# jseppanen/azalea

Hardware: AMD Instinct MI355X
Metric: mcts_sims_per_sec (higher is better)
Workload: dtype f16x3 (fp32 operands split hi+lo f16, fp32 accumulate)

## Files before the change

### azalea_amd/csrc/net_kernels.hip

```cpp
#include "net_priv.h"
#include "tower_tiles.h"

#ifndef AZX_NET_ABLATE
#define AZX_NET_ABLATE 0
#endif
#ifndef AZX_SAT_TRACK
#define AZX_SAT_TRACK 1
#endif

#include <cmath>
#include <cstdio>
#include <cstdlib>
#include <cstring>
#include <map>
#include <string>
#include <type_traits>
#include <utility>
#include <vector>

typedef float f32x16 __attribute__((ext_vector_type(16)));

static thread_local std::string g_net_err;
const char *azx_net_error() { return g_net_err.c_str(); }

// ... 47 lines not shown
            Xb[(size_t)rows * LDW + ncells * LDW + c] = 0.0f;
        }
    }
    __syncthreads();

    const int li = lane & 31, lh = lane >> 5;
    int ry[MTW], rx[MTW];
    bool rvalid[MTW];
#pragma unroll
    for (int m = 0; m < MTW; ++m) {
        const int r = (ms * MTW + m) * 32 + li;
        rvalid[m] = r < ncells;
        ry[m] = r / N;
        rx[m] = r - ry[m] * N;
    }

    for (int layer = 0; layer < P.layers; ++layer) {
        const float *src = (layer & 1) ? Y : X;
        float *dst = (layer & 1) ? X : Y;
        f32x16 acc[MTW][NTW];
#pragma unroll
        for (int m = 0; m < MTW; ++m)
#pragma unroll
            for (int n = 0; n < NTW; ++n)
#pragma unroll
                for (int r = 0; r < 16; ++r) acc[m][n][r] = 0.0f;

        const float4 *wl = reinterpret_cast<const float4 *>(P.Wp) +
                           (size_t)layer * 9 * (C / 8) * NT * 64;
        for (int tap = 0; tap < 9; ++tap) {
            const int dy = tap / 3 - 1, dx = tap % 3 - 1;
            int aoff[MTW];
#pragma unroll
            for (int m = 0; m < MTW; ++m) {
                const int yy = ry[m] + dy, xx = rx[m] + dx;
                const bool ok = rvalid[m] && yy >= 0 && yy < N && xx >= 0 && xx < N;
                aoff[m] = (ok ? (yy * N + xx) : ncells) * LDW + 4 * lh;
            }
            const float4 *wt = wl + (size_t)tap * (C / 8) * NT * 64;
#pragma unroll 2
            for (int q = 0; q < C / 8; ++q) {
                float4 bfrag[NTW];
#pragma unroll
                for (int n = 0; n < NTW; ++n)
                    bfrag[n] = wt[((size_t)q * NT + (ns * NTW + n)) * 64 + lane];
                float4 afrag[MTW];
#pragma unroll
                for (int m = 0; m < MTW; ++m)
                    afrag[m] = *reinterpret_cast<const float4 *>(src + aoff[m] + 8 * q);
#pragma unroll
                for (int m = 0; m < MTW; ++m)
#pragma unroll
                    for (int n = 0; n < NTW; ++n) {
                        acc[m][n] = __builtin_amdgcn_mfma_f32_32x32x2f32(afrag[m].x, bfrag[n].x, acc[m][n], 0, 0, 0);
                        acc[m][n] = __builtin_amdgcn_mfma_f32_32x32x2f32(afrag[m].y, bfrag[n].y, acc[m][n], 0, 0, 0);
                        acc[m][n] = __builtin_amdgcn_mfma_f32_32x32x2f32(afrag[m].z, bfrag[n].z, acc[m][n], 0, 0, 0);
                        acc[m][n] = __builtin_amdgcn_mfma_f32_32x32x2f32(afrag[m].w, bfrag[n].w, acc[m][n], 0, 0, 0);
                    }
            }
        }
        const bool residual = (layer & 1) != 0;
#pragma unroll
        for (int n = 0; n < NTW; ++n) {
            const int co = (ns * NTW + n) * 32 + li;
            const float bb = P.bias[layer * C + co];
#pragma unroll
            for (int m = 0; m < MTW; ++m) {
#pragma unroll
                for (int r = 0; r < 16; ++r) {
                    const int row = (ms * MTW + m) * 32 + (r & 3) + 8 * (r >> 2) + 4 * lh;
                    if (row < ncells) {
                        float v = acc[m][n][r] + bb;
                        if (residual) v += dst[row * LDW + co];
                        dst[row * LDW + co] = fmaxf(v, 0.0f);
                    }
                }
            }
        }
        __syncthreads();
    }

    for (int b = 0; b < BPB; ++b) {
        const int e = e0 + b;
        if (e >= n_eval) break;
        const float *Xb = lds + (size_t)b * 2 * rows * LDW;
        float4 *out = reinterpret_cast<float4 *>(act_out + (size_t)e * ncells * C);
        for (int idx = tid; idx < ncells * (C / 4); idx += 256) {
            const int pos = idx / (C / 4), c4 = idx - pos * (C / 4);
            out[idx] = *reinterpret_cast<const float4 *>(Xb + pos * LDW + 4 * c4);
        }
    }
}


typedef _Float16 f16x8 __attribute__((ext_vector_type(8)));

__device__ __forceinline__ void split_f16(float v, _Float16 &hi, _Float16 &lo) {
    hi = (_Float16)v;
    lo = (_Float16)(v - (float)hi);
}
__device__ __forceinline__ void split2_f16(float a, float b, uint32_t &hpk, uint32_t &lpk) {
    float la, lb;
    asm("v_cvt_pk_f16_f32 %0, %1, %2" : "=v"(hpk) : "v"(a), "v"(b));
    asm("v_fma_mix_f32 %0, %1, -1.0, %2 op_sel_hi:[1,0,0]" : "=v"(la) : "v"(hpk), "v"(a));
    asm("v_fma_mix_f32 %0, %1, -1.0, %2 op_sel:[1,0,0] op_sel_hi:[1,0,0]" : "=v"(lb) : "v"(hpk), "v"(b));
    asm("v_cvt_pk_f16_f32 %0, %1, %2" : "=v"(lpk) : "v"(la), "v"(lb));
#if AZX_LO_BITS < 10
    lpk = (lpk + LO_RND * 0x10001u) & (LO_MASK * 0x10001u);
#endif
}

#ifdef AZX_NET_STAMP
__device__ unsigned long long g_tower_stamp[10];
#define NT_DECL unsigned long long nt_last = __builtin_amdgcn_s_memtime(), nt_acc[8] = {0, 0, 0, 0, 0, 0, 0, 0}; const unsigned long long nt_rt0 = __builtin_amdgcn_s_memrealtime();
__device__ unsigned long long g_tower_trace[3 * 32768];
#define NT_MARK(r) { const unsigned long long nt_now = __builtin_amdgcn_s_memtime(); nt_acc[r] += nt_now - nt_last; nt_last = nt_now; }
#define NT_FLUSH if (tid == 0) { for (int r_ = 0; r_ < 7; ++r_) atomicAdd(&g_tower_stamp[r_], nt_acc[r_]); atomicAdd(&g_tower_stamp[7], 1ull); atomicAdd(&g_tower_stamp[8], __builtin_amdgcn_s_memrealtime() - nt_rt0); \
    if (blockIdx.x < 32768) { const unsigned hw = __builtin_amdgcn_s_getreg((31 << 11) | 4), xc = __builtin_amdgcn_s_getreg((31 << 11) | 20); \
        g_tower_trace[3 * blockIdx.x] = ((unsigned long long)(xc & 0xf) << 8) | (((hw >> 13) & 7) << 5) | (((hw >> 12) & 1) << 4) | ((hw >> 8) & 0xf); \
        g_tower_trace[3 * blockIdx.x + 1] = nt_rt0; g_tower_trace[3 * blockIdx.x + 2] = __builtin_amdgcn_s_memrealtime(); } }
__device__ unsigned long long g_wide_stamp[10];
#define WT_FLUSH if (lane == 0) { for (int r_ = 0; r_ < 7; ++r_) atomicAdd(&g_wide_stamp[r_], nt_acc[r_]); atomicAdd(&g_wide_stamp[7], 1ull); \
    atomicAdd(&g_wide_stamp[8], __builtin_amdgcn_s_memrealtime() - nt_rt0); }
#else
#define NT_DECL
#define NT_MARK(r)
#define NT_FLUSH
#define WT_FLUSH
#endif

#ifndef F16X3_BPB
#define F16X3_BPB 2
#endif
#ifndef AZX_S16_FENCE
#define AZX_S16_FENCE 1
#endif
typedef float f32x4 __attribute__((ext_vector_type(4)));

__global__ __launch_bounds__(F16X3_BPB * 128, 2) void k_tower_f16x3_s16(NetDev P, const uint8_t *__restrict__ ev_board,
                                                                        const int32_t *__restrict__ n_eval_ptr,
                                                                        int n_eval_host, float *__restrict__ act_out,
                                                                        float *__restrict__ hfeat) {
    constexpr int C = 64, ROWB = 272, MT = 4, NT = 4;
    extern __shared__ __align__(16) unsigned char smem[];
    const int n_eval = n_eval_ptr ? *n_eval_ptr : n_eval_host;
    const int e0 = blockIdx.x * F16X3_BPB;
    if (e0 >= n_eval) return;
    const int tid = threadIdx.x, lane = tid & 63, wave = __builtin_amdgcn_readfirstlane(tid >> 6);
    NT_DECL
    const int wb = wave >> 1, wh = wave & 1;
    const int N = P.N, ncells = P.ncells;
    const int e = e0 + wb;
    const bool live = e < n_eval;
    const int board_b = 128 * ROWB;
    const int zero_off = 0;
    const int x_off = 2 * ROWB + wb * board_b;
    unsigned char *X = smem + x_off;
    const int li = lane & 15, lh = lane >> 4;
    const int lrow = li < 8 ? li ^ 4 : li;
    const int lchunk = 128 * (lh & 1) + 16 * (lh >> 1);

    constexpr int LT = AZX_TOWER_LIGHT_SLOT;
    static_assert(LT == MT - 1, "the k-loop skips the lagging last tile");
    const uint8_t *tmap = P.tile_map + 64 * wave + lrow;
    const uint32_t skip = __builtin_amdgcn_readfirstlane((uint32_t)(P.tile_skip >> (9 * wave)) & 0x1ffu);
    unsigned long long tapok = 0ull;
    int rbase[MT], cell0_[MT];
#pragma unroll
    for (int m = 0; m < MT; ++m) {
        const int L = tmap[16 * m];
        const int r = L & 127;
        const int ry = r / N, rx = r - ry * N;
        cell0_[m] = r < ncells ? 2 * ROWB + (L >> 7) * board_b + 121 * ROWB + ry * (N + 2) + rx : -1;
        rbase[m] = 2 * ROWB + L * ROWB + lchunk;
#pragma unroll
        for (int tap = 0; tap < 9; ++tap) {
            const int yy = ry + tap / 3 - 1, xx = rx + tap % 3 - 1;
            if (r < ncells && yy >= 0 && yy < N && xx >= 0 && xx < N) tapok |= 1ull << (tap * 4 + m);
        }
    }
    uint32_t tapok_lo = (uint32_t)tapok, tapok_hi = (uint32_t)(tapok >> 32);
    auto act_offset = [&](int tap, int m) -> int {
        const int delta = ((tap / 3 - 1) * N + (tap % 3 - 1)) * ROWB;
        const uint32_t word = tap < 8 ? tapok_lo : tapok_hi;
        const int mask = (int)(word << (31 - ((tap * 4 + m) & 31))) >> 31;
        return (mask | 0xF0) & (rbase[m] + delta);
    };

    f32x4 res[MT][NT];
    auto load_bias = [&](const float *bias, float4 (&b4)[NT]) {
#pragma unroll
        for (int n = 0; n < NT; ++n) b4[n] = *reinterpret_cast<const float4 *>(bias + 16 * n + 4 * lh);
    };
    float satmax = 0.f;
    auto epilogue = [&](f32x4 (&acc)[MT][NT], const float4 (&bias4)[NT], auto kind_tag) {
        constexpr int kind = decltype(kind_tag)::value;
#pragma unroll
        for (int n = 0; n < NT; ++n) {
            const float4 b4 = bias4[n];
            const float bv[4] = {b4.x, b4.y, b4.z, b4.w};
#pragma unroll
            for (int m = 0; m < MT; ++m) {
                float v4[4];
#pragma unroll
                for (int j = 0; j < 4; ++j) {
                    float v = acc[m][n][j] + bv[j];
                    if (kind == 1) v += res[m][n][j];
                    v = fmaxf(v, 0.0f);
                    if (kind != 0) res[m][n][j] = v;
                    v4[j] = v;
                }
                if (AZX_SAT_TRACK) {
                    satmax = fmaxf(fmaxf(satmax, v4[0]), fmaxf(v4[1], fmaxf(v4[2], v4[3])));
                    asm volatile("" : "+v"(satmax));
                }
                uint2 h4, l4;
                split2_f16(v4[0], v4[1], h4.x, l4.x);
                split2_f16(v4[2], v4[3], h4.y, l4.y);
                unsigned char *pw = smem + rbase[m] + (112 * (lh >> 1) - 120 * (lh & 1)) + 16 * n;
                *reinterpret_cast<uint2 *>(pw) = h4;
                *reinterpret_cast<uint2 *>(pw + 64) = l4;
            }
        }
    };

    {
        const int NH = N + 2;
        unsigned char *cells = X + 121 * ROWB;
        const uint8_t *bd = ev_board + (size_t)(live ? e : n_eval - 1) * AZX_CELL_STRIDE;
        if (wh == 0) {
            for (int i = lane; i < NH * NH; i += 64) {
                const int y = i / NH - 1, x = i - (y + 1) * NH - 1;
                cells[i] = (y >= 0 && y < N && x >= 0 && x < N) ? bd[y * N + x] : (uint8_t)3;
            }
        }
        for (int i = tid; i < 2 * ROWB / 4; i += F16X3_BPB * 128) reinterpret_cast<uint32_t *>(smem + zero_off)[i] = 0u;
        __syncthreads();
        f32x4 acc[MT][NT];
#pragma unroll
        for (int m = 0; m < MT; ++m)
#pragma unroll
            for (int n = 0; n < NT; ++n) acc[m][n] = f32x4{0.f, 0.f, 0.f, 0.f};
        const uint4 *ws = reinterpret_cast<const uint4 *>(P.Ws16);
        f16x8 wfh[NT], wfl[NT];
#pragma unroll
        for (int n = 0; n < NT; ++n) {
            const uint4 qh = ws[(n * 2) * 64 + lane], ql = ws[(n * 2 + 1) * 64 + lane];
            wfh[n] = *reinterpret_cast<const f16x8 *>(&qh);
            wfl[n] = *reinterpret_cast<const f16x8 *>(&ql);
        }
#pragma unroll
        for (int m = 0; m < MT; ++m) {
            uint32_t onehot = 0u;
            if (cell0_[m] >= 0) {
                const unsigned char *c0 = smem + cell0_[m];
#pragma unroll
                for (int tap = 0; tap < 9; ++tap) {
                    const uint32_t v = c0[(tap / 3) * NH + tap % 3];
                    onehot |= (v < 3u ? 1u : 0u) << (3 * tap + v);
                }
            }
            const uint32_t byte = (onehot >> (8 * lh)) & 0xffu;
            uint4 q;
            q.x = ((byte >> 0) & 1u) * 0x3C00u | ((byte >> 1) & 1u) * 0x3C000000u;
            q.y = ((byte >> 2) & 1u) * 0x3C00u | ((byte >> 3) & 1u) * 0x3C000000u;
            q.z = ((byte >> 4) & 1u) * 0x3C00u | ((byte >> 5) & 1u) * 0x3C000000u;
            q.w = ((byte >> 6) & 1u) * 0x3C00u | ((byte >> 7) & 1u) * 0x3C000000u;
            const f16x8 xf = *reinterpret_cast<const f16x8 *>(&q);
#pragma unroll
            for (int n = 0; n < NT; ++n) {
                acc[m][n] = __builtin_amdgcn_mfma_f32_16x16x32_f16(wfh[n], xf, acc[m][n], 0, 0, 0);
                acc[m][n] = __builtin_amdgcn_mfma_f32_16x16x32_f16(wfl[n], xf, acc[m][n], 0, 0, 0);
            }
        }
        float4 sb4[NT];
        load_bias(P.stem_b, sb4);
        __syncthreads();
        epilogue(acc, sb4, std::integral_constant<int, 2>{});
    }
    __syncthreads();
    NT_MARK(0)

    const uint4 *wsrc = reinterpret_cast<const uint4 *>(P.Wh16);
    int stage = 0;
    const int last_stage = P.layers * 18 - 1;
    f16x8 wh_[NT], wl_[NT];
    auto load_w = [&](int st, int nn, int part) {
        const uint4 qq = wsrc[(size_t)min(st, last_stage) * 512 + (nn * 2 + part) * 64 + lane];
        if (part) wl_[nn] = *reinterpret_cast<const f16x8 *>(&qq);
        else wh_[nn] = *reinterpret_cast<const f16x8 *>(&qq);
    };
#pragma unroll
    for (int i = 0; i < 4; ++i) load_w(0, i >> 1, i & 1);
    auto conv_layer = [&](int layer, auto residual_tag) {
        constexpr bool residual = decltype(residual_tag)::value;
        asm volatile("" : "+v"(tapok_lo), "+v"(tapok_hi), "+v"(rbase[0]), "+v"(rbase[1]), "+v"(rbase[2]), "+v"(rbase[3]));
        f32x4 acc[MT][NT];
#pragma unroll
        for (int m = 0; m < MT; ++m)
#pragma unroll
            for (int n = 0; n < NT; ++n) acc[m][n] = f32x4{0.f, 0.f, 0.f, 0.f};
        f16x8 xh[MT], xl[MT];
        auto load_x = [&](int tt, int mm, int part) {
            const unsigned char *pa = smem + act_offset(tt >> 1, mm) + (tt & 1) * 32 + part * 64;
            if (part) xl[mm] = *reinterpret_cast<const f16x8 *>(pa);
            else xh[mm] = *reinterpret_cast<const f16x8 *>(pa);
        };
        auto tap_skipped = [&](int tap) __attribute__((always_inline)) -> bool {
            uint32_t s = skip;
            asm volatile("" : "+s"(s));
            return (s >> tap) & 1u;
        };
        auto fence = [&](int q) __attribute__((always_inline)) {
#if AZX_S16_FENCE == 2
            __builtin_amdgcn_sched_barrier(0);
#elif AZX_S16_FENCE == 1
            if (q % 3 == 2) __builtin_amdgcn_sched_barrier(0);
#elif AZX_S16_FENCE == 3
            if (q % 6 == 5) __builtin_amdgcn_sched_barrier(0);
#elif AZX_S16_FENCE == 4
            if (q % 2 == 1) __builtin_amdgcn_sched_barrier(0);
#endif
        };
        auto mfma1 = [&](int h, int m, int j) __attribute__((always_inline)) {
            const int n = 2 * h + j / 3, p = j % 3;
            const f16x8 wv = p == 1 ? wl_[n] : wh_[n];
            const f16x8 xv = p == 2 ? xl[m] : xh[m];
            acc[m][n] = __builtin_amdgcn_mfma_f32_16x16x32_f16(wv, xv, acc[m][n], 0, 0, 0);
        };
#pragma unroll
        for (int m = 0; m < MT - 1; ++m) { load_x(0, m, 0); load_x(0, m, 1); }
#pragma unroll
        for (int t = 0; t < 18; ++t) {
#pragma unroll
            for (int h = 0; h < 2; ++h) {
                auto step_q = [&](int q) __attribute__((always_inline)) {
                    if (q == 1 || q == 4 || q == 7 || q == 10) {
                        const int idx = (q - 1) / 3;
                        if (h == 0) load_w(stage + t, 2 + (idx >> 1), idx & 1);
                        else load_w(stage + t + 1, idx >> 1, idx & 1);
                    } else if (h == 0 && (q == 13 || q == 16)) {
                        load_x(t, MT - 1, q == 16);
                    } else if (h == 1 && q >= 8 && (q % 6 == 2 || q % 6 == 5)) {
                        if (t + 1 < 18) load_x(t + 1, q / 6 - 1, q % 6 == 5);
                    }
                    mfma1(h, q / 6, q % 6);
                    fence(q);
                };
#pragma unroll
                for (int q = 0; q < 6 * LT; ++q) step_q(q);
                if (!tap_skipped(t >> 1)) {
#pragma unroll
                    for (int q = 6 * LT; q < 24; ++q) step_q(q);
                } else if (h == 1 && t + 1 < 18) {
                    load_x(t + 1, MT - 2, 0);
                    load_x(t + 1, MT - 2, 1);
                }
            }
        }
        stage += 18;
        float4 lb4[NT];
        load_bias(P.bias + layer * C, lb4);
        NT_MARK(2)
        __syncthreads();
        NT_MARK(3)
        epilogue(acc, lb4, std::integral_constant<int, residual ? 1 : 0>{});
        NT_MARK(4)
        __syncthreads();
        NT_MARK(5)
    };
    for (int blk = 0; blk < P.blocks; ++blk) {
        conv_layer(2 * blk, std::false_type{});
        conv_layer(2 * blk + 1, std::true_type{});
    }

    if (hfeat != nullptr) {
        const uint4 *whd = reinterpret_cast<const uint4 *>(P.Whd16);
        f16x8 ah[2], al[2];
#pragma unroll
        for (int ks = 0; ks < 2; ++ks) {
            const uint4 qh = whd[(ks * 2) * 64 + lane], ql = whd[(ks * 2 + 1) * 64 + lane];
            ah[ks] = *reinterpret_cast<const f16x8 *>(&qh);
            al[ks] = *reinterpret_cast<const f16x8 *>(&ql);
        }
        const float4 hb = *reinterpret_cast<const float4 *>(P.hbias16 + 4 * lh);
        const float hbv[4] = {hb.x, hb.y, hb.z, hb.w};
#pragma unroll
        for (int m = 0; m < MT; ++m) {
            f32x4 hacc = f32x4{0.f, 0.f, 0.f, 0.f};
#pragma unroll
            for (int ks = 0; ks < 2; ++ks) {
                const unsigned char *pa = smem + rbase[m] + ks * 32;
                const f16x8 xh = *reinterpret_cast<const f16x8 *>(pa), xl = *reinterpret_cast<const f16x8 *>(pa + 64);
                hacc = __builtin_amdgcn_mfma_f32_16x16x32_f16(ah[ks], xh, hacc, 0, 0, 0);
                hacc = __builtin_amdgcn_mfma_f32_16x16x32_f16(al[ks], xh, hacc, 0, 0, 0);
                hacc = __builtin_amdgcn_mfma_f32_16x16x32_f16(ah[ks], xl, hacc, 0, 0, 0);
            }
            const int L = tmap[16 * m], row = L & 127, el = e0 + (L >> 7);
            if (el < n_eval && row < ncells) {
#pragma unroll
                for (int r = 0; r < 4; ++r) {
                    const int o = 4 * lh + r;
                    if (o < 6) hfeat[((size_t)el * 6 + o) * ncells + row] = fmaxf(hacc[r] + hbv[r], 0.0f);
                }
            }
        }
    }
    if (act_out != nullptr) {
#pragma unroll
        for (int m = 0; m < MT; ++m) {
            const int L = tmap[16 * m], row = L & 127, el = e0 + (L >> 7);
            float *out = act_out + (size_t)el * ncells * C;
            if (el < n_eval && row < ncells) {
#pragma unroll
                for (int n = 0; n < NT; ++n)
                    *reinterpret_cast<float4 *>(out + row * C + 16 * n + 4 * lh) =
                        make_float4(res[m][n][0], res[m][n][1], res[m][n][2], res[m][n][3]);
            }
        }
    }
    if (satmax > 65504.0f) atomicOr(P.sat_flag, 1u);
    NT_MARK(6)
    NT_FLUSH
}

__global__ __launch_bounds__(F16X3_BPB * 128, 2) void k_tower_f16_s16(NetDev P, const uint8_t *__restrict__ ev_board,
                                                                      const int32_t *__restrict__ n_eval_ptr,
                                                                      int n_eval_host, float *__restrict__ hfeat) {
    constexpr int C = 64, ROWB = 272, MT = 4, NT = 4;
    extern __shared__ __align__(16) unsigned char smem[];
    const int n_eval = n_eval_ptr ? *n_eval_ptr : n_eval_host;
    const int e0 = blockIdx.x * F16X3_BPB;
    if (e0 >= n_eval) return;
    const int tid = threadIdx.x, lane = tid & 63, wave = __builtin_amdgcn_readfirstlane(tid >> 6);
    const int wb = wave >> 1, wh = wave & 1;
    const int N = P.N, ncells = P.ncells;
    const int e = e0 + wb;
    const bool live = e < n_eval;
    const int board_b = 128 * ROWB;
    const int zero_off = 0;
    const int x_off = 2 * ROWB + wb * board_b;
    unsigned char *X = smem + x_off;
    const int li = lane & 15, lh = lane >> 4;
    const int lrow = li < 8 ? li ^ 4 : li;
    const int lchunk = 128 * (lh & 1) + 16 * (lh >> 1);

    unsigned long long tapok = 0ull;
    int rbase[MT], ry_[MT], rx_[MT];
#pragma unroll
    for (int m = 0; m < MT; ++m) {
        const int r = 64 * wh + 16 * m + lrow;
        const int ry = r / N, rx = r - ry * N;
        ry_[m] = ry;
        rx_[m] = rx;
        rbase[m] = x_off + r * ROWB + lchunk;
#pragma unroll
        for (int tap = 0; tap < 9; ++tap) {
            const int yy = ry + tap / 3 - 1, xx = rx + tap % 3 - 1;
            if (r < ncells && yy >= 0 && yy < N && xx >= 0 && xx < N) tapok |= 1ull << (tap * 4 + m);
        }
    }
    uint32_t tapok_lo = (uint32_t)tapok, tapok_hi = (uint32_t)(tapok >> 32);
    auto act_offset = [&](int tap, int m) -> int {
        const int delta = ((tap / 3 - 1) * N + (tap % 3 - 1)) * ROWB;
        const uint32_t word = tap < 8 ? tapok_lo : tapok_hi;
        const int mask = (int)(word << (31 - ((tap * 4 + m) & 31))) >> 31;
        return (mask | 0xF0) & (rbase[m] + delta);
    };

    f32x4 res[MT][NT];
    auto load_bias = [&](const float *bias, float4 (&b4)[NT]) {
#pragma unroll
        for (int n = 0; n < NT; ++n) b4[n] = *reinterpret_cast<const float4 *>(bias + 16 * n + 4 * lh);
    };
    float satmax = 0.f;
    auto epilogue = [&](f32x4 (&acc)[MT][NT], const float4 (&bias4)[NT], auto kind_tag) {
        constexpr int kind = decltype(kind_tag)::value;
#pragma unroll
        for (int n = 0; n < NT; ++n) {
            const float4 b4 = bias4[n];
            const float bv[4] = {b4.x, b4.y, b4.z, b4.w};
#pragma unroll
            for (int m = 0; m < MT; ++m) {
                float v4[4];
#pragma unroll
                for (int j = 0; j < 4; ++j) {
                    float v = acc[m][n][j] + bv[j];
                    if (kind == 1) v += res[m][n][j];
                    v = fmaxf(v, 0.0f);
                    if (kind != 0) res[m][n][j] = v;
                    v4[j] = v;
                }
                if (AZX_SAT_TRACK) satmax = fmaxf(fmaxf(satmax, v4[0]), fmaxf(v4[1], fmaxf(v4[2], v4[3])));
                uint2 h4;
                asm("v_cvt_pk_f16_f32 %0, %1, %2" : "=v"(h4.x) : "v"(v4[0]), "v"(v4[1]));
                asm("v_cvt_pk_f16_f32 %0, %1, %2" : "=v"(h4.y) : "v"(v4[2]), "v"(v4[3]));
                unsigned char *pw = X + (64 * wh + 16 * m + lrow) * ROWB + 128 * (lh >> 1) + 16 * n + 8 * (lh & 1);
                *reinterpret_cast<uint2 *>(pw) = h4;
            }
        }
    };

    {
        const int NH = N + 2;
        unsigned char *cells = X + 121 * ROWB;
        const uint8_t *bd = ev_board + (size_t)(live ? e : n_eval - 1) * AZX_CELL_STRIDE;
        if (wh == 0) {
            for (int i = lane; i < NH * NH; i += 64) {
                const int y = i / NH - 1, x = i - (y + 1) * NH - 1;
                cells[i] = (y >= 0 && y < N && x >= 0 && x < N) ? bd[y * N + x] : (uint8_t)3;
            }
        }
        for (int i = tid; i < 2 * ROWB / 4; i += F16X3_BPB * 128) reinterpret_cast<uint32_t *>(smem + zero_off)[i] = 0u;
        __syncthreads();
        f32x4 acc[MT][NT];
#pragma unroll
        for (int m = 0; m < MT; ++m)
#pragma unroll
            for (int n = 0; n < NT; ++n) acc[m][n] = f32x4{0.f, 0.f, 0.f, 0.f};
        const uint4 *ws = reinterpret_cast<const uint4 *>(P.Ws16);
        f16x8 wf[NT];
#pragma unroll
        for (int n = 0; n < NT; ++n) {
            const uint4 qh = ws[(n * 2) * 64 + lane];
            wf[n] = *reinterpret_cast<const f16x8 *>(&qh);
        }
// ... 1107 lines not shown
    }
    if (part == 0 && t < ncells) {
        const float bias = P.mfcb[t];
#pragma unroll
        for (int b = 0; b < HEADS_BPB; ++b) {
            const float logit = accm[b] + bias;
            lg[b][t] = logit;
            if (b < nb) logit_out[(size_t)(e0 + b) * AZX_CELL_STRIDE + t] = logit;
        }
    }
    __syncthreads();
    if (tid < nb) {
        float acc = 0.f;
        for (int i = 0; i < 64; ++i) acc += h2[i][tid] * P.fc3w[i];
        value_out[e0 + tid] = tanhf(acc + P.fc3b[0]);
    }
    if (!prior_out) return;
    const int lane = tid & 63, wave = tid >> 6;
    for (int b = wave; b < nb; b += 3 * HEADS_KSPLIT) {
        const int e = e0 + b;
        float x[3];
        bool legal[3];
        float mx = -INFINITY;
#pragma unroll
        for (int s = 0; s < 3; ++s) {
            const int cell = s * 64 + lane;
            legal[s] = cell < ncells && ev_board[(size_t)e * AZX_CELL_STRIDE + cell] == 0;
            x[s] = legal[s] ? lg[b][cell] : -INFINITY;
            mx = fmaxf(mx, x[s]);
        }
        mx = wave_max(mx);
        float sum = 0.f;
#pragma unroll
        for (int s = 0; s < 3; ++s) sum += legal[s] ? expf(x[s] - mx) : 0.f;
        const float lse = mx + logf(wave_sum(sum));
        const int flip = ev_flip[e];
#pragma unroll
        for (int s = 0; s < 3; ++s) {
            const int cell = s * 64 + lane;
            if (cell < ncells) {
                const int uc = (flip & 2) ? ncells - 1 - cell : cell;
                int oc = uc;
                if (flip & 1) {
                    const int i = uc / N, j = uc - i * N;
                    oc = (N - 1 - j) * N + (N - 1 - i);
                }
                prior_out[(size_t)e * AZX_CELL_STRIDE + oc] = legal[s] ? expf(x[s] - lse) : 0.f;
            }
        }
    }
}



static int raise_lds_limits() {
    const int cap = 160 * 1024;
    const void *fns[] = {(const void *)k_tower_f16x3_s16, (const void *)k_tower_f16_s16, (const void *)k_conv_wide_f16x3_s16,
                         (const void *)k_conv_wide_f16_s16,
                         (const void *)k_tower_mfma<64, 4, 2, 1, 2>, (const void *)k_tower_mfma<64, 6, 1, 2, 2>,
                         (const void *)k_tower_mfma<32, 6, 2, 2, 1>, (const void *)k_heads_mfma, (const void *)k_heads};
    for (const void *f : fns)
        if (hipFuncSetAttribute(f, hipFuncAttributeMaxDynamicSharedMemorySize, cap) != hipSuccess)
            return nfail(AZX_EHIP, "net: raising a tower kernel's dynamic LDS limit failed");
    return AZX_OK;
}

bool azx_net_has_fused_tower(int N, int blocks, int chans) { return chans == 64 && N * N <= 121 && blocks >= 1; }
static bool has_wide_tower(int N, int chans) { return chans % 128 == 0 && N * N <= 192; }
bool azx_net_has_f16_tower(int N, int blocks, int chans) {
    return azx_net_has_fused_tower(N, blocks, chans) || (has_wide_tower(N, chans) && blocks >= 1);
}

int azx_net_create(AzxNet **out, int N, int blocks, int chans, int max_evals, int tower_f16, hipStream_t st) {
    if (N < 2 || N > AZX_MAX_BOARD) return nfail(AZX_EINVAL, "net: board size out of range");
    if (blocks < 0 || chans < 1) return nfail(AZX_EINVAL, "net: bad num_blocks/base_chans");
    if (int rc = raise_lds_limits()) return rc;
    AzxNet *net = new AzxNet();
    memset(&net->d, 0, sizeof net->d);
    net->d.N = N;
    net->d.ncells = N * N;
    net->d.C = chans;
    net->d.blocks = blocks;
    net->d.layers = 2 * blocks;
    net->max_evals = max_evals;
    net->stream = st;
    const int ncells = N * N;
    const char *force = getenv("AZX_TOWER");
    const bool want_fp32 = force && !strcmp(force, "fp32");
    const bool fused = azx_net_has_fused_tower(N, blocks, chans);
    const bool has_f16 = azx_net_has_f16_tower(N, blocks, chans);
    if (tower_f16 && (!has_f16 || want_fp32)) {
        delete net;
        return nfail(AZX_EINVAL, want_fp32 ? "net: the plain-f16 tower was asked for (AZX_FLAG_TOWER_F16) but AZX_TOWER=fp32 forces the fp32 tower"
                                           : "net: the plain-f16 tower (AZX_FLAG_TOWER_F16) exists for the fused tower's shapes (64 channels, at most "
                                             "121 cells) and the wide tower's (a multiple of 128 channels) only, with at least one block");
    }
    const bool want_f16 = tower_f16 || (force && !strcmp(force, "f16"));
    if (fused && !want_fp32) { net->tower_variant = 4; net->tower_f16 = want_f16; }
    else if (chans == 64 && ncells <= 128) net->tower_variant = 1;
    else if (chans == 64 && ncells <= 192) net->tower_variant = 2;
    else if (chans == 32 && ncells <= 192) net->tower_variant = 3;
    else if (has_wide_tower(N, chans) && !want_fp32) {
        net->tower_variant = 5;
        net->tower_f16 = want_f16 && blocks >= 1;
    }
    net->use_mfma = net->tower_variant != 0;
    { const char *v = getenv("AZX_WIDE_STREAMS"); net->opt_wsplit = std::min(4, std::max(1, v ? atoi(v) : 2)); }
    { const char *v = getenv("AZX_HEADS"); net->opt_heads_mfma = !(v && !strcmp(v, "valu")); }
    { const char *v = getenv("AZX_PACK"); net->pack_on_host = v && !strcmp(v, "host"); }
    const bool x3 = net->tower_variant == 4 && !net->tower_f16;
    AzxTowerTiles tiles;
    bool want_edge = true;
    { const char *v = getenv("AZX_TOWER_TILES"); want_edge = !(v && !strcmp(v, "rows")); }
    azx_tower_tiles_build(N, x3 && want_edge, &tiles);
    {
        char b[320];
        const char *tower = "k_stem_generic + k_conv_generic (VALU)";
        if (net->tower_variant == 4) tower = net->tower_f16 ? "k_tower_f16_s16" : "k_tower_f16x3_s16";
        else if (net->tower_variant == 5) tower = net->tower_f16 ? "k_stem_wide_f16 + k_conv_wide_f16_s16 per layer"
                                                                 : "k_stem_wide_f16x3 + k_conv_wide_f16x3_s16 per layer";
        else if (net->tower_variant == 1) tower = "k_tower_mfma<64,4,2,1,2> (fp32 MFMA)";
        else if (net->tower_variant == 2) tower = "k_tower_mfma<64,6,1,2,2> (fp32 MFMA)";
        else if (net->tower_variant == 3) tower = "k_tower_mfma<32,6,2,2,1> (fp32 MFMA)";
        const bool hm = net->tower_variant == 4 && net->opt_heads_mfma && ncells <= 128;
        snprintf(b, sizeof b, "%s + %s (%dx%d on %dx%d; AZX_TOWER=%s AZX_TOWER_TILES=%s AZX_WIDE_STREAMS=%d AZX_HEADS=%s AZX_PACK=%s)",
                 tower, hm ? "k_heads_mfma" : "k_heads", blocks, chans, N, N, want_fp32 ? "fp32" : net->tower_f16 ? "f16" : "default",
                 want_edge && (tiles.edge || !x3) ? "edge" : "rows",
                 net->opt_wsplit, net->opt_heads_mfma ? "mfma" : "valu", net->pack_on_host ? "host" : "device");
        net->info = b;
    }
    const size_t E = max_evals;
    net->act = nalloc<float>(net, E * ncells * chans);
    net->logit = nalloc<float>(net, E * AZX_CELL_STRIDE);
    if (net->tower_variant == 4) net->hfeat = nalloc<float>(net, E * 6 * ncells);
    net->hb_board = nalloc<uint8_t>(net, E * AZX_CELL_STRIDE);
    net->hb_flip = nalloc<int32_t>(net, E);
    net->hb_value = nalloc<float>(net, E);
    if (!net->use_mfma) {
        net->act2 = nalloc<float>(net, E * ncells * chans);
        net->act3 = nalloc<float>(net, E * ncells * chans);
    }
    if (net->tower_variant == 5) {
        net->wideX = nalloc<unsigned short>(net, E * ncells * chans * 2);
        net->wideY = nalloc<unsigned short>(net, E * ncells * chans * 2);
    }
    if (!net->act || !net->logit || !net->hb_board || !net->hb_flip || !net->hb_value ||
        (!net->use_mfma && (!net->act2 || !net->act3)) || (net->tower_variant == 5 && (!net->wideX || !net->wideY))) {
        azx_net_destroy(net);
        return nfail(AZX_ENOMEM, "net: hipMalloc failed");
    }
    const int bpb = net->tower_variant == 2 ? 1 : 2;
    net->lds_bytes = (size_t)bpb * 2 * (ncells + 1) * (chans + 4) * sizeof(float);
    if (net->tower_variant == 4) net->lds_bytes = (size_t)F16X3_BPB * 128 * 272 + 2 * 272;
    if (net->tower_variant == 5) net->lds_bytes = (size_t)(ncells + 2) * WIDE_ROWB;
    net->d.sat_flag = nalloc<uint32_t>(net, 4);
    if (x3) {
        uint8_t *tm = nalloc<uint8_t>(net, sizeof tiles.row);
        if (tm && hipMemcpy(tm, tiles.row, sizeof tiles.row, hipMemcpyHostToDevice) != hipSuccess) tm = nullptr;
        if (!tm) {
            azx_net_destroy(net);
            return nfail(AZX_ENOMEM, "net: the tower's tile map could not be put on the device");
        }
        net->d.tile_map = tm;
        for (int w = 0; w < 4; ++w) net->d.tile_skip |= (unsigned long long)(tiles.skip[w] & 0x1ffu) << (9 * w);
    }
    if (!net->d.sat_flag || hipDeviceSynchronize() != hipSuccess) {
        azx_net_destroy(net);
        return nfail(AZX_ENOMEM, "net: hipMalloc failed");
    }
    *out = net;
    return AZX_OK;
}

void azx_net_set_stream(AzxNet *net, hipStream_t st, const uint32_t *mask, int words) {
    if (!net) return;
    for (int i = 0; i < 3; ++i) {
        if (net->stream2[i]) { (void)hipStreamSynchronize(net->stream2[i]); (void)hipStreamDestroy(net->stream2[i]); }
        if (net->ev_join[i]) (void)hipEventDestroy(net->ev_join[i]);
        net->stream2[i] = nullptr;
        net->ev_join[i] = nullptr;
    }
    if (net->ev_fork) (void)hipEventDestroy(net->ev_fork);
    net->ev_fork = nullptr;
    net->streams_ok = false;
    net->cu_mask.assign(mask, mask + (mask ? words : 0));
    net->stream = st;
}

void azx_net_destroy(AzxNet *net) {
    if (net) {
        for (int i = 0; i < 3; ++i) {
            if (net->stream2[i]) { (void)hipStreamSynchronize(net->stream2[i]); (void)hipStreamDestroy(net->stream2[i]); }
            if (net->ev_join[i]) (void)hipEventDestroy(net->ev_join[i]);
            net->stream2[i] = nullptr;
            net->ev_join[i] = nullptr;
        }
        if (net->ev_fork) (void)hipEventDestroy(net->ev_fork);
        net->ev_fork = nullptr;
    }
#ifdef AZX_NET_STAMP
    {
        unsigned long long h[10] = {0};
        if (hipMemcpyFromSymbol(h, HIP_SYMBOL(g_wide_stamp), sizeof h) == hipSuccess && h[7]) {
            static const char *nm[6] = {"prologue (bias + residual, setup)", "barrier after staging", "k-loops (MFMA)", "epilogue (stores acknowledged)",
                                        "barrier before staging (skew)", "staging: requests, round trips, LDS writes"};
            unsigned long long tot = 0;
            for (int r = 0; r < 6; ++r) tot += h[r];
            fprintf(stderr, "k_conv_wide_f16x3_s16 stamps over %llu waves: %.0f cycles/wave, shader clock %.0f MHz during the kernel\n",
                    h[7], (double)tot / h[7], h[8] ? 100.0 * (double)tot / (double)h[8] : 0.0);
            for (int r = 0; r < 6; ++r)
                fprintf(stderr, "  %-44s %6.1f%%  %9.0f cycles/wave\n", nm[r], 100.0 * h[r] / tot, (double)h[r] / h[7]);
            unsigned long long z[10] = {0};
            (void)hipMemcpyToSymbol(HIP_SYMBOL(g_wide_stamp), z, sizeof z);
        }
    }
    {
        unsigned long long h[10] = {0};
        if (hipMemcpyFromSymbol(h, HIP_SYMBOL(g_tower_stamp), sizeof h) == hipSuccess && h[7]) {
            static const char *nm[7] = {"stem", "residual load/setup", "k-loop (MFMA)", "barrier after k-loop",
                                        "epilogue", "barrier after epilogue", "output store"};
            unsigned long long tot = 0;
            for (int r = 0; r < 7; ++r) tot += h[r];
            fprintf(stderr, "k_tower_f16x3_s16 stamps over %llu blocks: %.0f cycles/block, shader clock %.0f MHz during the kernel\n",
                    h[7], (double)tot / h[7], h[8] ? 100.0 * (double)tot / (double)h[8] : 0.0);
            for (int r = 0; r < 7; ++r)
                fprintf(stderr, "  %-24s %6.1f%%  %9.0f cycles/block\n", nm[r], 100.0 * h[r] / tot, (double)h[r] / h[7]);
            {
                std::vector<unsigned long long> tr(3 * 32768);
                (void)hipMemcpyFromSymbol(tr.data(), HIP_SYMBOL(g_tower_trace), tr.size() * sizeof(unsigned long long));
                std::map<unsigned long long, std::vector<std::pair<unsigned long long, unsigned long long>>> cu;
                unsigned long long t0 = ~0ull, t1 = 0;
                size_t nblk = 0;
                for (int b = 0; b < 32768; ++b)
                    if (tr[3 * b + 2]) {
                        cu[tr[3 * b]].push_back({tr[3 * b + 1], tr[3 * b + 2]});
                        t0 = std::min(t0, tr[3 * b + 1]);
                        t1 = std::max(t1, tr[3 * b + 2]);
                        ++nblk;
                    }
                double busy = 0, mn = 1e30, mx = 0, lastend_min = 1e30, lastend_max = 0;
                size_t cmin = 1 << 30, cmax = 0;
                for (auto &kv : cu) {
                    double b = 0, le = 0;
                    for (auto &iv : kv.second) { b += (double)(iv.second - iv.first); le = std::max(le, (double)(iv.second - t0)); }
                    busy += b; mn = std::min(mn, b); mx = std::max(mx, b);
                    cmin = std::min(cmin, kv.second.size()); cmax = std::max(cmax, kv.second.size());
                    lastend_min = std::min(lastend_min, le); lastend_max = std::max(lastend_max, le);
                }
                fprintf(stderr, "  last launch: %zu blocks on %zu CUs, span %.1f us, blocks/CU %zu..%zu, mean resident blocks/CU %.2f, "
                        "per-CU block-time %.0f..%.0f us, CU finish %.0f..%.0f us\n", nblk, cu.size(), (t1 - t0) / 100.0, cmin, cmax,
                        busy / ((double)(t1 - t0) * cu.size()), mn / 100.0, mx / 100.0, lastend_min / 100.0, lastend_max / 100.0);
            }
            int nb = -1;
            (void)hipOccupancyMaxActiveBlocksPerMultiprocessor(&nb, (const void *)k_tower_f16x3_s16, F16X3_BPB * 128, net->lds_bytes);
            hipFuncAttributes fa;
            memset(&fa, 0, sizeof fa);
            (void)hipFuncGetAttributes(&fa, (const void *)k_tower_f16x3_s16);
            fprintf(stderr, "  runtime occupancy: %d blocks/CU (dynamic LDS %zu B, static %zu B, %d VGPRs, max threads %d)\n", nb,
                    net->lds_bytes, (size_t)fa.sharedSizeBytes, fa.numRegs, fa.maxThreadsPerBlock);
        }
    }
#endif
    if (!net) return;
    for (void *p : net->allocs) (void)hipFree(p);
    if (net->raw_tab_host) (void)hipHostFree((void *)net->raw_tab_host);
    if (net->wmax_host) (void)hipHostFree((void *)net->wmax_host);
    delete net;
}

bool azx_net_ready(const AzxNet *net) { return net && net->ready; }


static void run_net(AzxNet *net, const uint8_t *boards, const int32_t *flip, const int32_t *n_eval_ptr,
                    int n_host, int max_n, float *logit, float *value, float *prior, hipStream_t st, size_t row0 = 0) {
    const NetDev &d = net->d;
    if (max_n <= 0) return;
    const size_t act_rows = row0 * d.ncells * d.C;
    float *const act = net->act + act_rows;
    float *const act2 = net->act2 ? net->act2 + act_rows : nullptr;
    float *const act3 = net->act3 ? net->act3 + act_rows : nullptr;
    float *const hfeat_rows = net->hfeat ? net->hfeat + row0 * 6 * d.ncells : nullptr;
    const float *hfeat = nullptr;
    if (net->use_mfma) {
        const size_t lds = net->lds_bytes;
        if (net->tower_variant == 4) {
            const dim3 grid((max_n + F16X3_BPB - 1) / F16X3_BPB), block(F16X3_BPB * 128);
            if (net->tower_f16) hipLaunchKernelGGL(k_tower_f16_s16, grid, block, lds, st, d, boards, n_eval_ptr, n_host, hfeat_rows);
            else hipLaunchKernelGGL(k_tower_f16x3_s16, grid, block, lds, st, d, boards, n_eval_ptr, n_host, (float *)nullptr, hfeat_rows);
            hfeat = hfeat_rows;
        } else if (net->tower_variant == 5) {
            const dim3 grid(max_n, d.C / 128), block(256);
            const auto k_stem = net->tower_f16 ? k_stem_wide_f16 : k_stem_wide_f16x3;
            const auto k_conv = net->tower_f16 ? k_conv_wide_f16_s16 : k_conv_wide_f16x3_s16;
            hipLaunchKernelGGL(k_stem, grid, block, 0, st, d, boards, net->wideX,
                               d.blocks == 0 ? net->act : (float *)nullptr, n_eval_ptr, n_host);
            const int wsplit = net->opt_wsplit;
            {
                int parts = wsplit;
                if (parts > 1 && !net->ev_fork) {
                    bool ok = hipEventCreateWithFlags(&net->ev_fork, hipEventDisableTiming) == hipSuccess;
                    for (int i = 0; i < 3 && ok; ++i)
                        ok = (net->cu_mask.empty() ? hipStreamCreateWithFlags(&net->stream2[i], hipStreamNonBlocking)
                                                   : hipExtStreamCreateWithCUMask(&net->stream2[i], (uint32_t)net->cu_mask.size(), net->cu_mask.data())) == hipSuccess &&
                             hipEventCreateWithFlags(&net->ev_join[i], hipEventDisableTiming) == hipSuccess;
                    net->streams_ok = ok;
                }
// ... 146 lines not shown
```

### azalea_amd/csrc/tower_tiles.h

```cpp
#pragma once
#include <stdint.h>

#define AZX_TOWER_LIGHT_SLOT 3

struct AzxTowerTiles {
    uint8_t row[256];
    uint32_t skip[4];
    int edge;
};

static inline bool azx_tile_tap_is_padding(int N, int L, int tap) {
    const int cell = L & 127;
    if (cell >= N * N) return true;
    const int y = cell / N + tap / 3 - 1, x = cell % N + tap % 3 - 1;
    return y < 0 || y >= N || x < 0 || x >= N;
}

static inline void azx_tower_tiles_rows(AzxTowerTiles *t) {
    for (int i = 0; i < 256; ++i) t->row[i] = (uint8_t)i;
    for (int w = 0; w < 4; ++w) t->skip[w] = 0u;
    t->edge = 0;
}

static inline void azx_tile_slot_keys(int L, int tile_row, int *k1, int *k2) {
    const bool a = (tile_row & 4) == 0;
    *k1 = (L + (a ? 8 : 0)) & 15;
    *k2 = (L + (a ? 0 : 8)) & 15;
}

static inline void azx_tower_tiles_build(int N, int edge, AzxTowerTiles *t) {
    azx_tower_tiles_rows(t);
    if (!edge || N < 2 || N * N > 121) return;
    const int ncells = N * N;
    int cls[256];
    for (int L = 0; L < 256; ++L) {
        const int cell = L & 127, y = cell / N, x = cell % N;
        cls[L] = cell >= ncells ? 5 : y == 0 ? 0 : y == N - 1 ? 1 : x == 0 ? 2 : x == N - 1 ? 3 : 4;
    }
    bool used[256] = {false};
    int light[4][16];
    for (int c = 0; c < 4; ++c) {
        int nres[16] = {0}, chosen[16];
        for (int k = 0; k < 16; ++k) {
            int best = -1;
            for (int pass = 0; pass < 2 && best < 0; ++pass)
                for (int L = 0; L < 256; ++L)
                    if (!used[L] && cls[L] == (pass ? 5 : c) && (best < 0 || nres[L & 15] < nres[best & 15])) best = L;
            if (best < 0) { azx_tower_tiles_rows(t); return; }
            used[best] = true;
            ++nres[best & 15];
            chosen[k] = best;
        }
        int n1[16] = {0}, n2[16] = {0};
        bool taken[16] = {false};
        for (int k = 0; k < 16; ++k) {
            int best = -1, best_cost = 0;
            for (int r = 0; r < 16; ++r) {
                if (taken[r]) continue;
                int k1, k2;
                azx_tile_slot_keys(chosen[k], r, &k1, &k2);
                const int cost = n1[k1] + n2[k2];
                if (best < 0 || cost < best_cost) { best = r; best_cost = cost; }
            }
            int k1, k2;
            azx_tile_slot_keys(chosen[k], best, &k1, &k2);
            ++n1[k1];
            ++n2[k2];
            taken[best] = true;
            light[c][best] = chosen[k];
        }
    }
    int next = 0;
    for (int w = 0; w < 4; ++w)
        for (int m = 0; m < 4; ++m)
            for (int r = 0; r < 16; ++r) {
                if (m == AZX_TOWER_LIGHT_SLOT) { t->row[64 * w + 16 * m + r] = (uint8_t)light[w][r]; continue; }
                while (used[next]) ++next;
                t->row[64 * w + 16 * m + r] = (uint8_t)next++;
            }
    for (int w = 0; w < 4; ++w) {
        uint32_t mask = 0u;
        for (int tap = 0; tap < 9; ++tap) {
            bool all = true;
            for (int r = 0; r < 16; ++r) all = all && azx_tile_tap_is_padding(N, t->row[64 * w + 16 * AZX_TOWER_LIGHT_SLOT + r], tap);
            if (all) mask |= 1u << tap;
        }
        t->skip[w] = mask;
    }
    t->edge = 1;
}
```

Before: 5.400 million.

## Pad second board in LDS and rebalance tile rows to cut bank conflicts

Inserts an 8-row gap between the two boards' activation buffers in LDS and rebuilds the tile map so every 16-row tile, including the non-light ones, spreads its LDS rows evenly across residues mod 16. This is meant to reduce LDS bank conflicts on the A-operand loads. It also turns the per-block lambda pair into a single layer loop that picks the residual epilogue at runtime through an opaque scalar test, which shrinks code size, and it restructures the skipped-tap prefetch. It costs a little extra LDS per block and adds a runtime branch on the epilogue.

```diff
diff --git a/azalea_amd/csrc/net_kernels.hip b/azalea_amd/csrc/net_kernels.hip
--- a/azalea_amd/csrc/net_kernels.hip
+++ b/azalea_amd/csrc/net_kernels.hip
@@ -223,7 +223,7 @@
     const int N = P.N, ncells = P.ncells;
     const int e = e0 + wb;
     const bool live = e < n_eval;
-    const int board_b = 128 * ROWB;
+    const int board_b = (128 + AZX_TOWER_BOARD_GAP) * ROWB;
     const int zero_off = 0;
     const int x_off = 2 * ROWB + wb * board_b;
     unsigned char *X = smem + x_off;
@@ -243,7 +243,7 @@
         const int r = L & 127;
         const int ry = r / N, rx = r - ry * N;
         cell0_[m] = r < ncells ? 2 * ROWB + (L >> 7) * board_b + 121 * ROWB + ry * (N + 2) + rx : -1;
-        rbase[m] = 2 * ROWB + L * ROWB + lchunk;
+        rbase[m] = 2 * ROWB + (L + AZX_TOWER_BOARD_GAP * (L >> 7)) * ROWB + lchunk;
 #pragma unroll
         for (int tap = 0; tap < 9; ++tap) {
             const int yy = ry + tap / 3 - 1, xx = rx + tap % 3 - 1;
@@ -363,8 +363,7 @@
     };
 #pragma unroll
     for (int i = 0; i < 4; ++i) load_w(0, i >> 1, i & 1);
-    auto conv_layer = [&](int layer, auto residual_tag) {
-        constexpr bool residual = decltype(residual_tag)::value;
+    for (int layer = 0; layer < 2 * P.blocks; ++layer) {
         asm volatile("" : "+v"(tapok_lo), "+v"(tapok_hi), "+v"(rbase[0]), "+v"(rbase[1]), "+v"(rbase[2]), "+v"(rbase[3]));
         f32x4 acc[MT][NT];
 #pragma unroll
@@ -423,9 +422,12 @@
                 if (!tap_skipped(t >> 1)) {
 #pragma unroll
                     for (int q = 6 * LT; q < 24; ++q) step_q(q);
-                } else if (h == 1 && t + 1 < 18) {
-                    load_x(t + 1, MT - 2, 0);
-                    load_x(t + 1, MT - 2, 1);
+                }
+                if (h == 1 && t + 1 < 18) {
+                    if (tap_skipped(t >> 1)) {
+                        load_x(t + 1, MT - 2, 0);
+                        load_x(t + 1, MT - 2, 1);
+                    }
                 }
             }
         }
@@ -435,14 +437,16 @@
         NT_MARK(2)
         __syncthreads();
         NT_MARK(3)
-        epilogue(acc, lb4, std::integral_constant<int, residual ? 1 : 0>{});
+        auto second_conv = [&]() __attribute__((always_inline)) -> bool {
+            uint32_t s = (uint32_t)layer;
+            asm volatile("" : "+s"(s));
+            return s & 1u;
+        };
+        if (!second_conv()) epilogue(acc, lb4, std::integral_constant<int, 0>{});
+        if (second_conv()) epilogue(acc, lb4, std::integral_constant<int, 1>{});
         NT_MARK(4)
         __syncthreads();
         NT_MARK(5)
-    };
-    for (int blk = 0; blk < P.blocks; ++blk) {
-        conv_layer(2 * blk, std::false_type{});
-        conv_layer(2 * blk + 1, std::true_type{});
     }
 
     if (hfeat != nullptr) {
@@ -1856,6 +1860,7 @@
     const int bpb = net->tower_variant == 2 ? 1 : 2;
     net->lds_bytes = (size_t)bpb * 2 * (ncells + 1) * (chans + 4) * sizeof(float);
     if (net->tower_variant == 4) net->lds_bytes = (size_t)F16X3_BPB * 128 * 272 + 2 * 272;
+    if (x3) net->lds_bytes += (size_t)AZX_TOWER_BOARD_GAP * 272;
     if (net->tower_variant == 5) net->lds_bytes = (size_t)(ncells + 2) * WIDE_ROWB;
     net->d.sat_flag = nalloc<uint32_t>(net, 4);
     if (x3) {
diff --git a/azalea_amd/csrc/tower_tiles.h b/azalea_amd/csrc/tower_tiles.h
--- a/azalea_amd/csrc/tower_tiles.h
+++ b/azalea_amd/csrc/tower_tiles.h
@@ -22,62 +22,100 @@
     t->edge = 0;
 }
 
-static inline void azx_tile_slot_keys(int L, int tile_row, int *k1, int *k2) {
+#define AZX_TOWER_BOARD_GAP 8
+#define AZX_TOWER_LDS_ROWS (256 + AZX_TOWER_BOARD_GAP)
+static inline int azx_tile_lds_row(int L) { return L + AZX_TOWER_BOARD_GAP * (L >> 7); }
+
+static inline void azx_tile_slot_keys(int R, int tile_row, int *k1, int *k2) {
     const bool a = (tile_row & 4) == 0;
-    *k1 = (L + (a ? 8 : 0)) & 15;
-    *k2 = (L + (a ? 0 : 8)) & 15;
+    *k1 = (R + (a ? 8 : 0)) & 15;
+    *k2 = (R + (a ? 0 : 8)) & 15;
+}
+
+static inline void azx_tile_place(const int *chosen, int *out) {
+    int n1[16] = {0}, n2[16] = {0}, later[16], nlater = 0;
+    bool taken[16] = {false};
+    for (int k = 0; k < 16; ++k) {
+        const int R = azx_tile_lds_row(chosen[k]), r = R & 15;
+        if (taken[r]) { later[nlater++] = chosen[k]; continue; }
+        int k1, k2;
+        azx_tile_slot_keys(R, r, &k1, &k2);
+        ++n1[k1];
+        ++n2[k2];
+        taken[r] = true;
+        out[r] = chosen[k];
+    }
+    for (int k = 0; k < nlater; ++k) {
+        const int R = azx_tile_lds_row(later[k]);
+        int best = -1, best_cost = 0, k1, k2;
+        for (int r = 0; r < 16; ++r) {
+            if (taken[r]) continue;
+            azx_tile_slot_keys(R, r, &k1, &k2);
+            const int cost = n1[k1] + n2[k2];
+            if (best < 0 || cost < best_cost) { best = r; best_cost = cost; }
+        }
+        azx_tile_slot_keys(R, best, &k1, &k2);
+        ++n1[k1];
+        ++n2[k2];
+        taken[best] = true;
+        out[best] = later[k];
+    }
 }
 
 static inline void azx_tower_tiles_build(int N, int edge, AzxTowerTiles *t) {
     azx_tower_tiles_rows(t);
     if (!edge || N < 2 || N * N > 121) return;
     const int ncells = N * N;
-    int cls[256];
+    int cls[256], res[256];
     for (int L = 0; L < 256; ++L) {
         const int cell = L & 127, y = cell / N, x = cell % N;
         cls[L] = cell >= ncells ? 5 : y == 0 ? 0 : y == N - 1 ? 1 : x == 0 ? 2 : x == N - 1 ? 3 : 4;
+        res[L] = azx_tile_lds_row(L) & 15;
     }
     bool used[256] = {false};
-    int light[4][16];
+    int tile[16][16];
     for (int c = 0; c < 4; ++c) {
         int nres[16] = {0}, chosen[16];
         for (int k = 0; k < 16; ++k) {
             int best = -1;
             for (int pass = 0; pass < 2 && best < 0; ++pass)
                 for (int L = 0; L < 256; ++L)
-                    if (!used[L] && cls[L] == (pass ? 5 : c) && (best < 0 || nres[L & 15] < nres[best & 15])) best = L;
+                    if (!used[L] && cls[L] == (pass ? 5 : c) && (best < 0 || nres[res[L]] < nres[res[best]])) best = L;
             if (best < 0) { azx_tower_tiles_rows(t); return; }
             used[best] = true;
-            ++nres[best & 15];
+            ++nres[res[best]];
             chosen[k] = best;
         }
-        int n1[16] = {0}, n2[16] = {0};
-        bool taken[16] = {false};
-        for (int k = 0; k < 16; ++k) {
-            int best = -1, best_cost = 0;
-            for (int r = 0; r < 16; ++r) {
-                if (taken[r]) continue;
-                int k1, k2;
-                azx_tile_slot_keys(chosen[k], r, &k1, &k2);
-                const int cost = n1[k1] + n2[k2];
-                if (best < 0 || cost < best_cost) { best = r; best_cost = cost; }
-            }
-            int k1, k2;
-            azx_tile_slot_keys(chosen[k], best, &k1, &k2);
-            ++n1[k1];
-            ++n2[k2];
-            taken[best] = true;
-            light[c][best] = chosen[k];
+        azx_tile_place(chosen, tile[4 * c + AZX_TOWER_LIGHT_SLOT]);
+    }
+    int other[12], members[12][16], count[12], nres[12][16];
+    for (int w = 0, j = 0; w < 4; ++w)
+        for (int m = 0; m < 4; ++m)
+            if (m != AZX_TOWER_LIGHT_SLOT) other[j++] = 4 * w + m;
+    for (int j = 0; j < 12; ++j) {
+        count[j] = 0;
+        for (int rho = 0; rho < 16; ++rho) nres[j][rho] = 0;
+        for (int rho = 0; rho < 16; ++rho)
+            for (int L = 0; L < 256; ++L)
+                if (!used[L] && res[L] == rho) {
+                    used[L] = true;
+                    nres[j][rho] = 1;
+                    members[j][count[j]++] = L;
+                    break;
+                }
+    }
+    for (int j = 0; j < 12; ++j) {
+        while (count[j] < 16) {
+            int best = -1;
+            for (int L = 0; L < 256; ++L)
+                if (!used[L] && (best < 0 || nres[j][res[L]] < nres[j][res[best]])) best = L;
+            used[best] = true;
+            ++nres[j][res[best]];
+            members[j][count[j]++] = best;
         }
+        azx_tile_place(members[j], tile[other[j]]);
     }
-    int next = 0;
-    for (int w = 0; w < 4; ++w)
-        for (int m = 0; m < 4; ++m)
-            for (int r = 0; r < 16; ++r) {
-                if (m == AZX_TOWER_LIGHT_SLOT) { t->row[64 * w + 16 * m + r] = (uint8_t)light[w][r]; continue; }
-                while (used[next]) ++next;
-                t->row[64 * w + 16 * m + r] = (uint8_t)next++;
-            }
+    for (int i = 0; i < 256; ++i) t->row[i] = (uint8_t)tile[i >> 4][i & 15];
     for (int w = 0; w < 4; ++w) {
         uint32_t mask = 0u;
         for (int tap = 0; tap < 9; ++tap) {
```

Measured after the change: 5.526 million (median of 6 runs). +2.3%, better.
